# omerbt/Splice

Hardware: AMD Instinct MI355X
Metric: opt_steps_per_sec (higher is better)
Workload: dtype bf16

## Files before the change

### splice_amd/csrc/attn_bwd_x32.h

```cpp
#pragma once

constexpr int BX_SLOTS = 4;
constexpr int BX_Q_LDS = BX_SLOTS * 2 * 8192;
constexpr int BX_KV_LDS = BX_SLOTS * (2 * 8192 + 512);

__device__ __forceinline__ int bx_swz(int row) { return (((row >> 1) & 1) << 2) | (((row >> 3) & 1) << 1) | ((row >> 2) & 1); }

struct BxFrag {
    int rowa[4];
    int tra[2][2];
    __device__ __forceinline__ BxFrag(int lane) {
        const int q32 = lane & 31, hi = lane >> 5;
#pragma unroll
        for (int ks = 0; ks < 4; ++ks) rowa[ks] = q32 * 64 + (((2 * ks + hi) ^ bx_swz(q32)) << 3);
        const int m = lane & 15, dg = (lane >> 4) & 1;
#pragma unroll
        for (int db = 0; db < 2; ++db)
#pragma unroll
            for (int sec = 0; sec < 2; ++sec) {
                const int row = 8 * sec + 4 * hi + (m >> 2);
                tra[db][sec] = row * 64 + (((4 * db + 2 * dg + ((m >> 1) & 1)) ^ bx_swz(row)) << 3) + (m & 1) * 4;
            }
    }
};
__device__ __forceinline__ u32x4 bx_tr(const bf16_t* tile, const BxFrag& f, int db, int off) {
    typedef __attribute__((address_space(3))) tr_v4s lds_v4s;
    const tr_v4s lo = __builtin_amdgcn_ds_read_tr16_b64_v4i16((lds_v4s*)(tile + f.tra[db][0] + off));
    const tr_v4s hh = __builtin_amdgcn_ds_read_tr16_b64_v4i16((lds_v4s*)(tile + f.tra[db][1] + off));
    const uint2 x = __builtin_bit_cast(uint2, lo), y = __builtin_bit_cast(uint2, hh);
    return u32x4{x.x, x.y, y.x, y.y};
}
__device__ __forceinline__ void bx_mfma_seed(f32x16_t& d, const u32x4& a, const u32x4& b, const f32x16_t& c) {
    asm volatile("v_mfma_f32_32x32x16_bf16 %0, %1, %2, %3" : "=&v"(d) : "v"(a), "v"(b), "v"(c));
}
#define BX_SB __builtin_amdgcn_sched_barrier(0)

template <int NW>
struct BxDma {
    static constexpr int PIECES = 8 / NW;
    int wave, lr, chunk;
    uint32_t off[PIECES];
    __device__ __forceinline__ BxDma(int lane, int wave_, int ld, int coldelta) : wave(wave_) {
        lr = lane >> 3;
        const int pos = lane & 7;
        chunk = pos ^ ((((lr >> 1) & 1) << 2) | ((wave & 1) << 1) | ((lr >> 2) & 1));
#pragma unroll
        for (int i = 0; i < PIECES; ++i) off[i] = (uint32_t)((((wave + NW * i) * 8 + lr) * ld + chunk * 8 + coldelta) * 2);
    }
    __device__ __forceinline__ void tile(const bf16_t* base, int ld, int coldelta, int row0, int rows_total, uint32_t dst) const {
        if (row0 + 64 <= rows_total) {
            const bf16_t* tb = base + (size_t)row0 * ld;
#pragma unroll
            for (int i = 0; i < PIECES; ++i) pp_dma16(dst + i * (NW * 1024), off[i], tb);
        } else {
#pragma unroll
            for (int i = 0; i < PIECES; ++i) {
                int t = row0 + (wave + NW * i) * 8 + lr;
                t = t < rows_total ? t : rows_total - 1;
                pp_dma16(dst + i * (NW * 1024), (uint32_t)((t * ld + chunk * 8 + coldelta) * 2), base);
            }
        }
    }
};

template <int NW, bool FOLD>
__device__ __forceinline__ void attn_bwd_q_x32_body(const AttnArgs& a, int xb, int h, int b, bf16_t* bx_smem ) {
    constexpr int NL = 2 * (8 / NW);
    const int lane = threadIdx.x & 63, q32 = lane & 31, hi = lane >> 5;
    const int wave = __builtin_amdgcn_readfirstlane(threadIdx.x >> 6);
    const int ld = 3 * a.D;
    const int qbase = xb * (32 * NW) + wave * 32;
    const bool active = qbase < a.Tld;
    const bf16_t* pbase = a.qkv + (size_t)b * a.Tld * ld + h * 64;
    const int nt = (a.T + 63) / 64;
    const BxDma<NW> dk_(lane, wave, ld, a.D), dv_(lane, wave, ld, 2 * a.D);
    const BxFrag fr(lane);
    const uint32_t lds0 = (uint32_t)(size_t)(__attribute__((address_space(3))) bf16_t*)bx_smem + (uint32_t)wave * 1024u;
    auto issue = [&](int tile, int slot) __attribute__((always_inline)) {
        const uint32_t dst = __builtin_amdgcn_readfirstlane(lds0 + (uint32_t)slot * 16384u);
        dk_.tile(pbase, ld, a.D, tile * 64, a.Tld, dst);
        dv_.tile(pbase, ld, 2 * a.D, tile * 64, a.Tld, dst + 8192u);
    };
    issue(0, 0);
    if (nt > 1) issue(1, 1);
    if (nt > 2) issue(2, 2);

    const int qidx = qbase + q32;
    const int qc = qidx < a.Tld ? qidx : a.Tld - 1;
    u32x4 qf[4], dof[4];
    {
        const bf16_t* pq = pbase + (size_t)qc * ld + hi * 8;
        const bf16_t* pd = a.dout + ((size_t)b * a.Tld + qc) * a.D + h * 64 + hi * 8;
#pragma unroll
        for (int ks = 0; ks < 4; ++ks) { qf[ks] = ld16v(pq + ks * 16); dof[ks] = ld16v(pd + ks * 16); }
    }
    const float lse_q = a.lse[((size_t)b * a.H + h) * a.Tld + qc];
    const float del_q = a.delta[((size_t)b * a.H + h) * a.Tld + qc];
    const float c2 = a.scale * LOG2E;
    f32x16_t negl, negd, dq[2], s[2], dp[2];
    const f32x16_t zero16 = {0.f, 0.f, 0.f, 0.f, 0.f, 0.f, 0.f, 0.f, 0.f, 0.f, 0.f, 0.f, 0.f, 0.f, 0.f, 0.f};
#pragma unroll
    for (int r = 0; r < 16; ++r) { negl[r] = -lse_q; negd[r] = -del_q; dq[0][r] = dq[1][r] = 0.f; s[0][r] = s[1][r] = dp[0][r] = dp[1][r] = 0.f; }
    u32x4 kf[4], vf[4];
    auto read_rows = [&](const bf16_t* K, int blk) __attribute__((always_inline)) {
#pragma unroll
        for (int ks = 0; ks < 4; ++ks) { kf[ks] = lds16(K + fr.rowa[ks] + blk * 2048); vf[ks] = lds16(K + 4096 + fr.rowa[ks] + blk * 2048); }
    };
    auto sdp = [&](f32x16_t& sx, f32x16_t& dx, int ks) __attribute__((always_inline)) {
        if (ks == 0) {
            if (FOLD) bx_mfma_seed(sx, kf[0], qf[0], negl); else sx = mfma32(kf[0], qf[0], zero16);
            bx_mfma_seed(dx, vf[0], dof[0], negd);
        } else { sx = mfma32(kf[ks], qf[ks], sx); dx = mfma32(vf[ks], dof[ks], dx); }
    };
    pp_wait_dma<0>();
    asm volatile("" : "+v"(qf[0]), "+v"(qf[1]), "+v"(qf[2]), "+v"(qf[3]), "+v"(dof[0]), "+v"(dof[1]), "+v"(dof[2]), "+v"(dof[3]));
    pp_barrier();
    if (active) {
        read_rows(bx_smem, 0);
#pragma unroll
        for (int ks = 0; ks < 4; ++ks) sdp(s[0], dp[0], ks);
        read_rows(bx_smem, 1);
    }
    int slot = 0;
    auto body = [&](auto TAILC, int t) __attribute__((always_inline)) {
        constexpr bool TAIL = decltype(TAILC)::value;
        const int s1 = (slot + 1) & 3, s3 = (slot + 3) & 3;
        if (!TAIL || t + 2 < nt) pp_wait_dma<NL>(); else pp_wait_dma<0>();
        asm volatile("s_waitcnt lgkmcnt(0)" ::: "memory");
        pp_barrier();
        if (!TAIL || t + 3 < nt) issue(t + 3, s3);
        if (active) {
            const bf16_t* Kt = bx_smem + slot * 8192;
            const bf16_t* Kn = bx_smem + s1 * 8192;
#pragma unroll
            for (int blk = 0; blk < 2; ++blk) {
                f32x16_t& sc = s[blk];
                f32x16_t& dc = dp[blk];
                f32x16_t& sn = s[blk ^ 1];
                f32x16_t& dn = dp[blk ^ 1];
                if (TAIL && t * 64 + 64 > a.T) {
#pragma unroll
                    for (int r = 0; r < 16; ++r) sc[r] = t * 64 + 32 * blk + 8 * (r >> 2) + 4 * hi + (r & 3) < a.T ? sc[r] : NEG_BIG;
                }
                float g[16];
                u32x4 dsb[2], ktf[2][2];
                auto va = [&](int r0, int n) __attribute__((always_inline)) {
#pragma unroll
                    for (int r = r0; r < r0 + n; ++r) {
                        const float p = FOLD ? __builtin_amdgcn_exp2f(sc[r]) : __builtin_amdgcn_exp2f(__builtin_fmaf(sc[r], c2, -lse_q));
                        g[r] = p * dc[r];
                    }
                    asm volatile("" : "+v"(g[r0]), "+v"(g[r0 + n - 1]));
                };
                auto cv = [&](int kk) __attribute__((always_inline)) {
                    const float* pp = &g[kk * 8];
                    dsb[kk] = u32x4{pack2bf(pp[0], pp[1]), pack2bf(pp[2], pp[3]), pack2bf(pp[4], pp[5]), pack2bf(pp[6], pp[7])};
                    pp_opaque(dsb[kk]);
                };
                auto rt = [&](int kk, int db) __attribute__((always_inline)) {
                    ktf[kk][db] = bx_tr(Kt, fr, db, blk * 2048 + kk * 1024);
                };
                BX_SB;
                sdp(sn, dn, 0); BX_SB; va(0, 4); rt(0, 0); BX_SB;
                sdp(sn, dn, 1); BX_SB; va(4, 4); cv(0); rt(0, 1); BX_SB;
                sdp(sn, dn, 2); BX_SB; va(8, 4); rt(1, 0); BX_SB;
                sdp(sn, dn, 3); BX_SB; va(12, 4); cv(1); rt(1, 1); BX_SB;
                const bf16_t* Kr = blk == 0 ? Kn : Kn;
#pragma unroll
                for (int kk = 0; kk < 2; ++kk)
#pragma unroll
                    for (int db = 0; db < 2; ++db) {
                        dq[db] = mfma32(ktf[kk][db], dsb[kk], dq[db]);
                        BX_SB;
                        const int ks = kk * 2 + db;
                        kf[ks] = lds16(Kr + fr.rowa[ks] + blk * 2048); vf[ks] = lds16(Kr + 4096 + fr.rowa[ks] + blk * 2048);
                        BX_SB;
                    }
            }
        }
        slot = s1;
    };
    {
        std::false_type MAIN; std::true_type TAILT;
        int t = 0;
        for (; t + 4 < nt; ++t) body(MAIN, t);
        for (; t < nt; ++t) body(TAILT, t);
    }
    if (!active || qidx >= a.Tld) return;
    bf16_t* op = a.dqkv + ((size_t)b * a.Tld + qidx) * ld + h * 64 + hi * 4;
#pragma unroll
    for (int db = 0; db < 2; ++db)
#pragma unroll
        for (int j = 0; j < 4; ++j)
            *reinterpret_cast<uint2*>(op + db * 32 + j * 8) = uint2{pack2bf(dq[db][4 * j] * a.scale, dq[db][4 * j + 1] * a.scale),
                                                                    pack2bf(dq[db][4 * j + 2] * a.scale, dq[db][4 * j + 3] * a.scale)};
}

template <int NW>
__device__ __forceinline__ void attn_bwd_kv_x32_body(const AttnArgs& a, int xb, int h, int b, bf16_t* bx_smem ) {
    constexpr int SLOT = 2 * 4096 + 256;
    static_assert(NW >= 2, "waves 0 and 1 move the lse / delta rows");
    const int lane = threadIdx.x & 63, k32 = lane & 31, hi = lane >> 5;
    const int wave = __builtin_amdgcn_readfirstlane(threadIdx.x >> 6);
    const int ld = 3 * a.D;
    const int kbase = xb * (32 * NW) + wave * 32;
    const bool active = kbase < a.Tld;
    const bf16_t* pbase = a.qkv + (size_t)b * a.Tld * ld + h * 64;
    const bf16_t* dobase = a.dout + (size_t)b * a.Tld * a.D + h * 64;
    const float* lse = a.lse + ((size_t)b * a.H + h) * a.Tld;
    const float* dl = a.delta + ((size_t)b * a.H + h) * a.Tld;
    const int nblk = a.Tld / 32, nt = (nblk + 1) / 2;
    const BxDma<NW> dq_(lane, wave, ld, 0), dd_(lane, wave, a.D, 0);
    const BxFrag fr(lane);
    const uint32_t ldsb = (uint32_t)(size_t)(__attribute__((address_space(3))) bf16_t*)bx_smem;
    const uint32_t lds0 = ldsb + (uint32_t)wave * 1024u;
    auto issue = [&](int tile, int slot) __attribute__((always_inline)) {
        const uint32_t dst = __builtin_amdgcn_readfirstlane(lds0 + (uint32_t)slot * (SLOT * 2));
        dq_.tile(pbase, ld, 0, tile * 64, a.Tld, dst);
        dd_.tile(dobase, a.D, 0, tile * 64, a.Tld, dst + 8192u);
        if (wave < 2) {
            const int r = tile * 64 + lane;
            const uint32_t voff = (uint32_t)((r < a.Tld ? r : a.Tld - 1) * 4);
            const uint32_t d2 = __builtin_amdgcn_readfirstlane(ldsb + (uint32_t)slot * (SLOT * 2) + 16384u + (uint32_t)wave * 256u);
            const float* src = wave == 0 ? lse : dl;
            asm volatile("s_mov_b32 m0, %0\n\ts_nop 0\n\tglobal_load_lds_dword %1, %2" ::"s"(d2), "v"(voff), "s"(src) : "memory");
        }
    };
    issue(0, 0);
    if (nt > 1) issue(1, 1);
    if (nt > 2) issue(2, 2);

    const int kidx = kbase + k32;
    const int kc = kidx < a.Tld ? kidx : a.Tld - 1;
    u32x4 kn[4], vn[4];
    {
        const bf16_t* pk = pbase + (size_t)kc * ld + a.D + hi * 8;
        const bf16_t* pv = pbase + (size_t)kc * ld + 2 * a.D + hi * 8;
#pragma unroll
        for (int ks = 0; ks < 4; ++ks) {
            kn[ks] = ld16v(pk + ks * 16); vn[ks] = ld16v(pv + ks * 16);
#pragma unroll
            for (int j = 0; j < 4; ++j) { kn[ks][j] ^= 0x80008000u; vn[ks][j] ^= 0x80008000u; }
        }
    }
    f32x16_t dkn[2], dv[2];
#pragma unroll
    for (int r = 0; r < 16; ++r) { dkn[0][r] = dkn[1][r] = dv[0][r] = dv[1][r] = 0.f; }
    u32x4 qr[4], dr[4];
    f32x16_t sx, dx;
    auto seeds = [&](const bf16_t* st, int blk) __attribute__((always_inline)) {
        const float* Ls = reinterpret_cast<const float*>(st + 8192);
#pragma unroll
        for (int j = 0; j < 4; ++j) {
            const f32x4 lv = *reinterpret_cast<const f32x4*>(Ls + 32 * blk + 8 * j + 4 * hi);
            const f32x4 ev = *reinterpret_cast<const f32x4*>(Ls + 64 + 32 * blk + 8 * j + 4 * hi);
#pragma unroll
            for (int i = 0; i < 4; ++i) { sx[4 * j + i] = lv[i]; dx[4 * j + i] = ev[i]; }
        }
    };
    auto rows = [&](const bf16_t* st, int blk) __attribute__((always_inline)) {
#pragma unroll
        for (int ks = 0; ks < 4; ++ks) { qr[ks] = lds16(st + fr.rowa[ks] + blk * 2048); dr[ks] = lds16(st + 4096 + fr.rowa[ks] + blk * 2048); }
    };
    pp_wait_dma<0>();
    asm volatile("" : "+v"(kn[0]), "+v"(kn[1]), "+v"(kn[2]), "+v"(kn[3]), "+v"(vn[0]), "+v"(vn[1]), "+v"(vn[2]), "+v"(vn[3]));
    pp_barrier();
    if (active) { rows(bx_smem, 0); seeds(bx_smem, 0); }
    int slot = 0;
    auto body = [&](auto TAILC, int t) __attribute__((always_inline)) {
        constexpr bool TAIL = decltype(TAILC)::value;
        const int s1 = (slot + 1) & 3, s3 = (slot + 3) & 3;
        if (!TAIL || t + 2 < nt) { if (wave < 2) pp_wait_dma<2 * (8 / NW) + 1>(); else pp_wait_dma<2 * (8 / NW)>(); } else pp_wait_dma<0>();
        asm volatile("s_waitcnt lgkmcnt(0)" ::: "memory");
        pp_barrier();
        if (!TAIL || t + 3 < nt) issue(t + 3, s3);
        if (active) {
            const bf16_t* st = bx_smem + slot * SLOT;
            const bf16_t* sn = bx_smem + s1 * SLOT;
#pragma unroll
            for (int blk = 0; blk < 2; ++blk) {
                if (TAIL && 2 * t + blk >= nblk) break;
                u32x4 dot[2][2], qt[2][2], pb[2], gb[2];
                float p[16], g[16];
#pragma unroll
                for (int ks = 0; ks < 4; ++ks) {
                    sx = mfma32(qr[ks], kn[ks], sx);
                    BX_SB;
                    {
                        if (ks < 2) { dot[ks][0] = bx_tr(st + 4096, fr, 0, blk * 2048 + ks * 1024); dot[ks][1] = bx_tr(st + 4096, fr, 1, blk * 2048 + ks * 1024); }
                        else { qt[ks - 2][0] = bx_tr(st, fr, 0, blk * 2048 + (ks - 2) * 1024); qt[ks - 2][1] = bx_tr(st, fr, 1, blk * 2048 + (ks - 2) * 1024); }
                    }
                    BX_SB;
                }
#pragma unroll
                for (int ks = 0; ks < 4; ++ks) {
                    dx = mfma32(dr[ks], vn[ks], dx);
                    BX_SB;
                    {
#pragma unroll
                        for (int r = 4 * ks; r < 4 * ks + 4; ++r) p[r] = __builtin_amdgcn_exp2f(-sx[r]);
                        if (ks & 1) {
                            const float* pp = &p[(ks >> 1) * 8];
                            pb[ks >> 1] = u32x4{pack2bf(pp[0], pp[1]), pack2bf(pp[2], pp[3]), pack2bf(pp[4], pp[5]), pack2bf(pp[6], pp[7])};
                            pp_opaque(pb[ks >> 1]);
                        } else asm volatile("" : "+v"(p[4 * ks]), "+v"(p[4 * ks + 3]));
                    }
                    BX_SB;
                }
#pragma unroll
                for (int i4 = 0; i4 < 4; ++i4) {
                    const int kk = i4 >> 1, db = i4 & 1;
                    dv[db] = mfma32(dot[kk][db], pb[kk], dv[db]);
                    BX_SB;
                    {
#pragma unroll
                        for (int r = 4 * i4; r < 4 * i4 + 4; ++r) g[r] = p[r] * dx[r];
                        if (i4 & 1) {
                            const float* pp = &g[(i4 >> 1) * 8];
                            gb[i4 >> 1] = u32x4{pack2bf(pp[0], pp[1]), pack2bf(pp[2], pp[3]), pack2bf(pp[4], pp[5]), pack2bf(pp[6], pp[7])};
                            pp_opaque(gb[i4 >> 1]);
                        } else asm volatile("" : "+v"(g[4 * i4]), "+v"(g[4 * i4 + 3]));
                    }
                    BX_SB;
                }
                const bf16_t* nx_st = blk == 0 ? st : sn;
                const int nx_blk = blk ^ 1;
#pragma unroll
                for (int i4 = 0; i4 < 4; ++i4) {
                    const int kk = i4 >> 1, db = i4 & 1;
                    dkn[db] = mfma32(qt[kk][db], gb[kk], dkn[db]);
                    BX_SB;
                    {
                        const float* Ls = reinterpret_cast<const float*>(nx_st + 8192);
                        qr[i4] = lds16(nx_st + fr.rowa[i4] + nx_blk * 2048);
                        dr[i4] = lds16(nx_st + 4096 + fr.rowa[i4] + nx_blk * 2048);
                        const f32x4 lv = *reinterpret_cast<const f32x4*>(Ls + 32 * nx_blk + 8 * i4 + 4 * hi);
                        const f32x4 ev = *reinterpret_cast<const f32x4*>(Ls + 64 + 32 * nx_blk + 8 * i4 + 4 * hi);
#pragma unroll
                        for (int i = 0; i < 4; ++i) { sx[4 * i4 + i] = lv[i]; dx[4 * i4 + i] = ev[i]; }
                    }
                    BX_SB;
                }
            }
        }
        slot = s1;
    };
    {
        std::false_type MAIN; std::true_type TAILT;
        int t = 0;
        for (; t + 4 < nt; ++t) body(MAIN, t);
        for (; t < nt; ++t) body(TAILT, t);
    }
    if (!active || kidx >= a.Tld) return;
    const float sk = kidx < a.T ? -a.scale : 0.f, sv = kidx < a.T ? 1.0f : 0.f;
    bf16_t* pk = a.dqkv + ((size_t)b * a.Tld + kidx) * ld + a.D + h * 64 + hi * 4;
    bf16_t* pv = a.dqkv + ((size_t)b * a.Tld + kidx) * ld + 2 * a.D + h * 64 + hi * 4;
#pragma unroll
    for (int db = 0; db < 2; ++db)
#pragma unroll
        for (int j = 0; j < 4; ++j) {
            *reinterpret_cast<uint2*>(pk + db * 32 + j * 8) = uint2{pack2bf(dkn[db][4 * j] * sk, dkn[db][4 * j + 1] * sk), pack2bf(dkn[db][4 * j + 2] * sk, dkn[db][4 * j + 3] * sk)};
            *reinterpret_cast<uint2*>(pv + db * 32 + j * 8) = uint2{pack2bf(dv[db][4 * j] * sv, dv[db][4 * j + 1] * sv), pack2bf(dv[db][4 * j + 2] * sv, dv[db][4 * j + 3] * sv)};
        }
}
#undef BX_SB

template <int NW>
__global__ __launch_bounds__(64 * NW) void attn_bwd_x32_kernel(AttnArgs a, int nx) {
    extern __shared__ __attribute__((aligned(16))) bf16_t bx_smem[];
    const int n = nx * a.H * a.B;
    const int lid = xcd_remap(blockIdx.x, 2 * n);
    const int pair = lid >> 1;
    const int xb = pair % nx, bh = pair / nx;
    const int h = bh % a.H, b = bh / a.H;
    if (lid & 1) attn_bwd_kv_x32_body<NW>(a, xb, h, b, bx_smem);
    else attn_bwd_q_x32_body<NW, true>(a, xb, h, b, bx_smem);
}
template <int NW>
__global__ __launch_bounds__(64 * NW) void attn_bwd_q_x32_kernel(AttnArgs a, int nx) {
    extern __shared__ __attribute__((aligned(16))) bf16_t bx_smem[];
    int xb, h, b;
    attn_block_coords(nx, a.H, a.B, xb, h, b);
    attn_bwd_q_x32_body<NW, true>(a, xb, h, b, bx_smem);
}
template <int NW>
__global__ __launch_bounds__(64 * NW) void attn_bwd_kv_x32_kernel(AttnArgs a, int nx) {
    extern __shared__ __attribute__((aligned(16))) bf16_t bx_smem[];
    int xb, h, b;
    attn_block_coords(nx, a.H, a.B, xb, h, b);
    attn_bwd_kv_x32_body<NW>(a, xb, h, b, bx_smem);
}
```

### splice_amd/csrc/attn_x32.h

```cpp
#pragma once
#include <type_traits>

template <int NW>
struct X32 {
    static constexpr int PIECES = 8 / NW;
    static constexpr int NL = 2 * PIECES;
    static constexpr int LDS_BYTES = 6 * 8192;
};

__device__ __forceinline__ void pp_dma16(uint32_t lds_byte, uint32_t voff, const void* sbase) {
    asm volatile("s_mov_b32 m0, %0\n\ts_nop 0\n\tglobal_load_lds_dwordx4 %1, %2" ::"s"(lds_byte), "v"(voff), "s"(sbase) : "memory");
}
template <int N>
__device__ __forceinline__ void pp_wait_dma() { asm volatile("s_waitcnt vmcnt(%0)" ::"n"(N) : "memory"); }
__device__ __forceinline__ void pp_barrier() {
    __builtin_amdgcn_sched_barrier(0);
    __builtin_amdgcn_s_barrier();
    __builtin_amdgcn_sched_barrier(0);
}
template <class V> __device__ __forceinline__ void pp_opaque(V& v) { asm volatile("" : "+v"(v)); }

typedef __attribute__((ext_vector_type(16))) float f32x16_t;
__device__ __forceinline__ f32x16_t mfma32(const u32x4& a, const u32x4& b, const f32x16_t& c) {
    return __builtin_amdgcn_mfma_f32_32x32x16_bf16(__builtin_bit_cast(bf16x8, a), __builtin_bit_cast(bf16x8, b), c, 0, 0, 0);
}
__device__ __forceinline__ float half2_max(float v) { return fmaxf(v, __shfl_xor(v, 32, 64)); }

__device__ __forceinline__ void x32_exact_rows(const AttnArgs& a, const bf16_t* pbase, int b, int h, int qidx, int hi, float c2) {
    const int ld = 3 * a.D;
    const int qc = qidx < a.Tld ? qidx : a.Tld - 1;
    float q[64], o[64];
    {
        const bf16_t* p = pbase + (size_t)qc * ld;
#pragma unroll
        for (int i = 0; i < 8; ++i) {
            const u32x4 v = ld16v(p + i * 8);
#pragma unroll
            for (int j = 0; j < 4; ++j) { q[i * 8 + 2 * j] = __uint_as_float(v[j] << 16) * c2; q[i * 8 + 2 * j + 1] = __uint_as_float(v[j] & 0xFFFF0000u) * c2; }
        }
    }
#pragma unroll
    for (int d = 0; d < 64; ++d) o[d] = 0.f;
    float m = NEG_BIG, l = 0.f;
    for (int key = hi; key < a.T; key += 2) {
        const bf16_t* kp = pbase + (size_t)key * ld + a.D;
        float sc = 0.f;
#pragma unroll
        for (int i = 0; i < 8; ++i) {
            const u32x4 v = ld16v(kp + i * 8);
#pragma unroll
            for (int j = 0; j < 4; ++j) {
                sc = __builtin_fmaf(q[i * 8 + 2 * j], __uint_as_float(v[j] << 16), sc);
                sc = __builtin_fmaf(q[i * 8 + 2 * j + 1], __uint_as_float(v[j] & 0xFFFF0000u), sc);
            }
        }
        const float mn = fmaxf(m, sc);
        const float alpha = __builtin_amdgcn_exp2f(m - mn), pk = __builtin_amdgcn_exp2f(sc - mn);
        m = mn;
        l = l * alpha + pk;
        const bf16_t* vp = pbase + (size_t)key * ld + 2 * a.D;
#pragma unroll
        for (int i = 0; i < 8; ++i) {
            const u32x4 v = ld16v(vp + i * 8);
#pragma unroll
            for (int j = 0; j < 4; ++j) {
                o[i * 8 + 2 * j] = __builtin_fmaf(pk, __uint_as_float(v[j] << 16), o[i * 8 + 2 * j] * alpha);
                o[i * 8 + 2 * j + 1] = __builtin_fmaf(pk, __uint_as_float(v[j] & 0xFFFF0000u), o[i * 8 + 2 * j + 1] * alpha);
            }
        }
    }
    const float m1 = __shfl_xor(m, 32, 64), l1 = __shfl_xor(l, 32, 64);
    const float mn = fmaxf(m, m1);
    const float a0 = __builtin_amdgcn_exp2f(m - mn), a1 = __builtin_amdgcn_exp2f(m1 - mn);
    const float lt = l * a0 + l1 * a1, inv = 1.0f / lt;
    bf16_t* op = a.out + ((size_t)b * a.Tld + qc) * a.D + h * 64;
#pragma unroll
    for (int d = 0; d < 64; ++d) {
        const float od = (o[d] * a0 + __shfl_xor(o[d], 32, 64) * a1) * inv;
        if (hi == (d >> 5) && qidx < a.Tld) op[d] = f2bf(od);
    }
    if (hi == 0 && qidx < a.Tld) a.lse[((size_t)b * a.H + h) * a.Tld + qidx] = mn + __builtin_amdgcn_logf(lt);
}

template <int NW, bool FOLD>
__global__ __launch_bounds__(64 * NW) void attn_fwd_x32_kernel(AttnArgs a, int nx) {
    extern __shared__ __attribute__((aligned(16))) bf16_t x32_smem[];
    constexpr int PIECES = X32<NW>::PIECES, NL = X32<NW>::NL;
    const int lane = threadIdx.x & 63;
    const int q32 = lane & 31, hi = lane >> 5;
    const int wave = __builtin_amdgcn_readfirstlane(threadIdx.x >> 6);
    int xb, h, b;
    attn_block_coords(nx, a.H, a.B, xb, h, b);
    const int ld = 3 * a.D;
    const int qbase = xb * (32 * NW) + wave * 32;
    const bool active = qbase < a.Tld;
    const bf16_t* pbase = a.qkv + (size_t)b * a.Tld * ld + h * 64;
    const int nt = (a.T + 63) / 64;

    const int lr = lane >> 3, pos = lane & 7;
    const int kchunk = pos ^ (((wave & 1) << 2) | (lr >> 1));
    const int vchunk = pos ^ (((lr >> 1) & 1) << 2);
    uint32_t koffs[PIECES], voffs[PIECES];
#pragma unroll
    for (int i = 0; i < PIECES; ++i) {
        const int row = (wave + NW * i) * 8 + lr;
        koffs[i] = (uint32_t)((row * ld + kchunk * 8 + a.D) * 2);
        voffs[i] = (uint32_t)((row * ld + vchunk * 8 + 2 * a.D) * 2);
    }
    const uint32_t lds0 = (uint32_t)(size_t)(__attribute__((address_space(3))) bf16_t*)x32_smem + (uint32_t)wave * 1024u;
    auto issue_tile = [&](const uint32_t (&offs)[PIECES], int chunk, int coldelta, int tile, uint32_t dst) __attribute__((always_inline)) {
        const int kt = tile * 64;
        if (kt + 64 <= a.Tld) {
            const bf16_t* tb = pbase + (size_t)kt * ld;
#pragma unroll
            for (int i = 0; i < PIECES; ++i) pp_dma16(dst + i * (NW * 1024), offs[i], tb);
        } else {
#pragma unroll
            for (int i = 0; i < PIECES; ++i) {
                int t = kt + (wave + NW * i) * 8 + lr;
                t = t < a.Tld ? t : a.Tld - 1;
                pp_dma16(dst + i * (NW * 1024), (uint32_t)((t * ld + chunk * 8 + coldelta) * 2), pbase);
            }
        }
    };
    auto issue_k = [&](int tile, int slot) __attribute__((always_inline)) { issue_tile(koffs, kchunk, a.D, tile, __builtin_amdgcn_readfirstlane(lds0 + (uint32_t)slot * 8192u)); };
    auto issue_v = [&](int tile, int slot) __attribute__((always_inline)) { issue_tile(voffs, vchunk, 2 * a.D, tile, __builtin_amdgcn_readfirstlane(lds0 + 3 * 8192u + (uint32_t)slot * 8192u)); };
    const char* kptr = reinterpret_cast<const char*>(pbase) + (size_t)4 * 64 * ld * 2;
    const char* vptr = reinterpret_cast<const char*>(pbase) + (size_t)2 * 64 * ld * 2;
    const size_t tile_bytes = (size_t)64 * ld * 2;
    auto issue_fast = [&](int s1, int s2) __attribute__((always_inline)) {
        const uint32_t kd = __builtin_amdgcn_readfirstlane(lds0 + (uint32_t)s1 * 8192u), vd = __builtin_amdgcn_readfirstlane(lds0 + 3 * 8192u + (uint32_t)s2 * 8192u);
#pragma unroll
        for (int i = 0; i < PIECES; ++i) pp_dma16(kd + i * (NW * 1024), koffs[i], kptr);
#pragma unroll
        for (int i = 0; i < PIECES; ++i) pp_dma16(vd + i * (NW * 1024), voffs[i], vptr);
    };
    issue_k(0, 0);
    issue_v(0, 0);
    if (nt > 1) { issue_k(1, 1); issue_v(1, 1); }
    if (nt > 2) issue_k(2, 2);

    u32x4 qf[4];
    const int qidx = qbase + q32;
    {
        const int qc = qidx < a.Tld ? qidx : a.Tld - 1;
        const bf16_t* p = pbase + (size_t)qc * ld + hi * 8;
#pragma unroll
        for (int ks = 0; ks < 4; ++ks) qf[ks] = ld16v(p + ks * 16);
    }
    int ka[4];
#pragma unroll
    for (int ks = 0; ks < 4; ++ks) ka[ks] = q32 * 64 + (((2 * ks + hi) ^ ((q32 >> 1) & 7)) << 3);
    int va[2];
    {
        const int m = lane & 15, dg = (lane >> 4) & 1;
#pragma unroll
        for (int db = 0; db < 2; ++db)
            va[db] = (4 * hi + (m >> 2)) * 64 + (((4 * db + 2 * dg + ((m >> 1) & 1)) ^ (((m >> 3) & 1) << 2)) << 3) + (m & 1) * 4;
    }
    float m_ref = 0.f, l = 0.f;
    f32x16_t o[2], sb[2][2], negm;
#pragma unroll
    for (int r = 0; r < 16; ++r) { o[0][r] = 0.f; o[1][r] = 0.f; sb[0][0][r] = sb[0][1][r] = sb[1][0][r] = sb[1][1][r] = 0.f; negm[r] = 0.f; }
    const float c2 = a.scale * LOG2E;
    const f32x16_t zero16 = {0.f, 0.f, 0.f, 0.f, 0.f, 0.f, 0.f, 0.f, 0.f, 0.f, 0.f, 0.f, 0.f, 0.f, 0.f, 0.f};
    u32x4 kf[2][4];
    auto read_k = [&](const bf16_t* Ks) __attribute__((always_inline)) {
#pragma unroll
        for (int kb = 0; kb < 2; ++kb)
#pragma unroll
            for (int ks = 0; ks < 4; ++ks) kf[kb][ks] = lds16(Ks + ka[ks] + kb * 2048);
    };
    auto scores = [&](f32x16_t (&s)[2], const f32x16_t& seed) __attribute__((always_inline)) {
#pragma unroll
        for (int kb = 0; kb < 2; ++kb) s[kb] = mfma32(kf[kb][0], qf[0], seed);
#pragma unroll
        for (int ks = 1; ks < 4; ++ks)
#pragma unroll
            for (int kb = 0; kb < 2; ++kb) s[kb] = mfma32(kf[kb][ks], qf[ks], s[kb]);
    };
    const bf16_t* Kring = x32_smem;
    const bf16_t* Vring = x32_smem + 3 * 4096;

    pp_wait_dma<0>();
    asm volatile("" : "+v"(qf[0]), "+v"(qf[1]), "+v"(qf[2]), "+v"(qf[3]));
    pp_barrier();
    if (active) {
        read_k(Kring);
        scores(sb[0], zero16);
        float mx = NEG_BIG;
#pragma unroll
        for (int kb = 0; kb < 2; ++kb)
#pragma unroll
            for (int r = 0; r < 16; ++r) {
                const bool valid = 32 * kb + 8 * (r >> 2) + 4 * hi + (r & 3) < a.T;
                mx = fmaxf(mx, valid ? sb[0][kb][r] : NEG_BIG);
            }
        m_ref = half2_max(mx) * (FOLD ? 1.0f : c2);
#pragma unroll
        for (int r = 0; r < 16; ++r) negm[r] = -m_ref;
        if (FOLD) scores(sb[0], negm);
        if (nt > 1) read_k(Kring + 4096);
    }
    asm volatile("s_waitcnt lgkmcnt(0)" ::: "memory");
    pp_barrier();
    if (nt > 3) issue_k(3, 0);

    int slot = 0;
#define X32_SB __builtin_amdgcn_sched_barrier(0)
    auto body = [&](auto PARC, auto TAILC, int t) __attribute__((always_inline)) {
        constexpr int PAR = decltype(PARC)::value;
        constexpr bool TAIL = decltype(TAILC)::value;
        f32x16_t (&s)[2] = sb[PAR];
        f32x16_t (&sn)[2] = sb[PAR ^ 1];
        const int s1 = slot == 2 ? 0 : slot + 1, s2 = slot == 0 ? 2 : slot - 1;
        if (!TAIL || t + 3 < nt) pp_wait_dma<NL>(); else pp_wait_dma<0>();
        asm volatile("s_waitcnt lgkmcnt(0)" ::: "memory");
        pp_barrier();
        if (!TAIL) issue_fast(s1, s2);
        else {
            if (t + 4 < nt) issue_k(t + 4, s1);
            if (t + 2 < nt) issue_v(t + 2, s2);
        }
        kptr += tile_bytes;
        vptr += tile_bytes;
        if (active) {
            const bf16_t* Vs = Vring + slot * 4096;
            const bf16_t* Kn = Kring + s2 * 4096;
            u32x4 vf[4][2], pb[4];
            float p[2][16];
            float pa[4] = {0.f, 0.f, 0.f, 0.f};
            const int kt = t * 64;
            if (TAIL && kt + 64 > a.T) {
#pragma unroll
                for (int kb = 0; kb < 2; ++kb)
#pragma unroll
                    for (int r = 0; r < 16; ++r) s[kb][r] = kt + 32 * kb + 8 * (r >> 2) + 4 * hi + (r & 3) < a.T ? s[kb][r] : NEG_BIG;
            }
            auto ex = [&](int kb, int r0, int n) __attribute__((always_inline)) {
#pragma unroll
                for (int r = r0; r < r0 + n; ++r) {
                    p[kb][r] = FOLD ? __builtin_amdgcn_exp2f(s[kb][r]) : __builtin_amdgcn_exp2f(__builtin_fmaf(s[kb][r], c2, -m_ref));
                    pa[r & 3] += p[kb][r];
                }
                asm volatile("" : "+v"(pa[0]), "+v"(pa[1]), "+v"(pa[2]), "+v"(pa[3]));
            };
            auto cv = [&](int kk) __attribute__((always_inline)) {
                const float* pp = &p[kk >> 1][(kk & 1) * 8];
                pb[kk] = u32x4{pack2bf(pp[0], pp[1]), pack2bf(pp[2], pp[3]), pack2bf(pp[4], pp[5]), pack2bf(pp[6], pp[7])};
                pp_opaque(pb[kk]);
            };
            auto rv = [&](int kk, int db) __attribute__((always_inline)) {
                typedef __attribute__((address_space(3))) tr_v4s lds_v4s;
                const tr_v4s lo = __builtin_amdgcn_ds_read_tr16_b64_v4i16((lds_v4s*)(Vs + va[db] + kk * 1024));
                const tr_v4s hh = __builtin_amdgcn_ds_read_tr16_b64_v4i16((lds_v4s*)(Vs + va[db] + kk * 1024 + 512));
                const uint2 x = __builtin_bit_cast(uint2, lo), y = __builtin_bit_cast(uint2, hh);
                vf[kk][db] = u32x4{x.x, x.y, y.x, y.y};
            };
            auto rk = [&](int kb, int ks) __attribute__((always_inline)) {
                kf[kb][ks] = lds16(Kn + ka[ks] + kb * 2048);
            };
            auto qk = [&](int kb, int ks) __attribute__((always_inline)) {
                if (ks == 0 && FOLD) asm volatile("v_mfma_f32_32x32x16_bf16 %0, %1, %2, %3" : "=&v"(sn[kb]) : "v"(kf[kb][0]), "v"(qf[0]), "v"(negm));
                else sn[kb] = mfma32(kf[kb][ks], qf[ks], ks == 0 ? zero16 : sn[kb]);
            };
            auto pv = [&](int kk, int db) __attribute__((always_inline)) {
                o[db] = mfma32(vf[kk][db], pb[kk], o[db]);
            };
            X32_SB;
            qk(0, 0); X32_SB; ex(0, 0, 3); rv(0, 0); X32_SB;
            qk(1, 0); X32_SB; ex(0, 3, 3); rv(0, 1); X32_SB;
            qk(0, 1); X32_SB; ex(0, 6, 2); cv(0); rv(1, 0); X32_SB;
            qk(1, 1); X32_SB; ex(0, 8, 3); rv(1, 1); X32_SB;
            qk(0, 2); X32_SB; ex(0, 11, 3); rv(2, 0); X32_SB;
            qk(1, 2); X32_SB; ex(0, 14, 2); cv(1); rv(2, 1); X32_SB;
            qk(0, 3); X32_SB; ex(1, 0, 3); rv(3, 0); X32_SB;
            qk(1, 3); X32_SB; ex(1, 3, 3); rv(3, 1); X32_SB;
            pv(0, 0); X32_SB; ex(1, 6, 2); cv(2); rk(0, 0); X32_SB;
            pv(0, 1); X32_SB; ex(1, 8, 3); rk(1, 0); X32_SB;
            pv(1, 0); X32_SB; ex(1, 11, 3); rk(0, 1); X32_SB;
            pv(1, 1); X32_SB; ex(1, 14, 2); cv(3); rk(1, 1); X32_SB;
            pv(2, 0); X32_SB; rk(0, 2); X32_SB;
            pv(2, 1); X32_SB; rk(1, 2); X32_SB;
            pv(3, 0); X32_SB; rk(0, 3); X32_SB;
            pv(3, 1); X32_SB; rk(1, 3); X32_SB;
            const float ps = (pa[0] + pa[1]) + (pa[2] + pa[3]);
            l += ps;
            if (__builtin_expect(__any(!(ps < ATTN_RESCALE_LIMIT)), 0)) {
                const bool mine = half2_max(!(ps < ATTN_RESCALE_LIMIT) ? 1.0f : 0.0f) > 0.f;
                const float lq = l + __shfl_xor(l, 32, 64);
                const float shift = mine ? __builtin_amdgcn_logf(lq) : 0.f;
                const float alpha = __builtin_amdgcn_exp2f(-shift);
                m_ref += shift;
                l *= alpha;
#pragma unroll
                for (int r = 0; r < 16; ++r) {
                    negm[r] = -m_ref; o[0][r] *= alpha; o[1][r] *= alpha;
                    if (FOLD) { sn[0][r] -= shift; sn[1][r] -= shift; }
                }
            }
        }
        slot = s1;
    };
    {
        std::integral_constant<int, 0> P0; std::integral_constant<int, 1> P1;
        std::false_type MAIN; std::true_type TAILT;
        int t = 0;
        for (; t + 6 < nt; t += 2) {
            body(P0, MAIN, t);
            body(P1, MAIN, t + 1);
        }
        for (; t < nt; t += 2) {
            body(P0, TAILT, t);
            if (t + 1 < nt) body(P1, TAILT, t + 1);
        }
    }
#undef X32_SB
    if (!active) return;
    const float lt = l + __shfl_xor(l, 32, 64);
    if (__builtin_expect(__any(!(lt > 0.25f && lt < 1.0e37f)), 0)) {
        x32_exact_rows(a, pbase, b, h, qidx, hi, FOLD ? 1.0f : c2);
        return;
    }
    if (qidx < a.Tld) {
        const float inv = 1.0f / lt;
        bf16_t* op = a.out + ((size_t)b * a.Tld + qidx) * a.D + h * 64 + hi * 4;
#pragma unroll
        for (int db = 0; db < 2; ++db)
#pragma unroll
            for (int j = 0; j < 4; ++j)
                *reinterpret_cast<uint2*>(op + db * 32 + j * 8) =
                    uint2{pack2bf(o[db][4 * j] * inv, o[db][4 * j + 1] * inv), pack2bf(o[db][4 * j + 2] * inv, o[db][4 * j + 3] * inv)};
        if (hi == 0) a.lse[((size_t)b * a.H + h) * a.Tld + qidx] = m_ref + __builtin_amdgcn_logf(lt);
    }
}
```

Measured before the change: 263.5.

## Widen attention output stores via permlane swap and overlap Q load with K/V DMA

```diff
diff --git a/splice_amd/csrc/attn_bwd_x32.h b/splice_amd/csrc/attn_bwd_x32.h
--- a/splice_amd/csrc/attn_bwd_x32.h
+++ b/splice_amd/csrc/attn_bwd_x32.h
@@ -186,14 +186,8 @@
         for (; t + 4 < nt; ++t) body(MAIN, t);
         for (; t < nt; ++t) body(TAILT, t);
     }
-    if (!active || qidx >= a.Tld) return;
-    bf16_t* op = a.dqkv + ((size_t)b * a.Tld + qidx) * ld + h * 64 + hi * 4;
-#pragma unroll
-    for (int db = 0; db < 2; ++db)
-#pragma unroll
-        for (int j = 0; j < 4; ++j)
-            *reinterpret_cast<uint2*>(op + db * 32 + j * 8) = uint2{pack2bf(dq[db][4 * j] * a.scale, dq[db][4 * j + 1] * a.scale),
-                                                                    pack2bf(dq[db][4 * j + 2] * a.scale, dq[db][4 * j + 3] * a.scale)};
+    if (!active) return;
+    pp_store_row(a.dqkv + ((size_t)b * a.Tld + qidx) * ld + h * 64 + hi * 8, dq, a.scale, qidx < a.Tld);
 }
 
 template <int NW>
@@ -351,17 +345,11 @@
         for (; t + 4 < nt; ++t) body(MAIN, t);
         for (; t < nt; ++t) body(TAILT, t);
     }
-    if (!active || kidx >= a.Tld) return;
+    if (!active) return;
     const float sk = kidx < a.T ? -a.scale : 0.f, sv = kidx < a.T ? 1.0f : 0.f;
-    bf16_t* pk = a.dqkv + ((size_t)b * a.Tld + kidx) * ld + a.D + h * 64 + hi * 4;
-    bf16_t* pv = a.dqkv + ((size_t)b * a.Tld + kidx) * ld + 2 * a.D + h * 64 + hi * 4;
-#pragma unroll
-    for (int db = 0; db < 2; ++db)
-#pragma unroll
-        for (int j = 0; j < 4; ++j) {
-            *reinterpret_cast<uint2*>(pk + db * 32 + j * 8) = uint2{pack2bf(dkn[db][4 * j] * sk, dkn[db][4 * j + 1] * sk), pack2bf(dkn[db][4 * j + 2] * sk, dkn[db][4 * j + 3] * sk)};
-            *reinterpret_cast<uint2*>(pv + db * 32 + j * 8) = uint2{pack2bf(dv[db][4 * j] * sv, dv[db][4 * j + 1] * sv), pack2bf(dv[db][4 * j + 2] * sv, dv[db][4 * j + 3] * sv)};
-        }
+    bf16_t* pk = a.dqkv + ((size_t)b * a.Tld + kidx) * ld + a.D + h * 64 + hi * 8;
+    pp_store_row(pk, dkn, sk, kidx < a.Tld);
+    pp_store_row(pk + a.D, dv, sv, kidx < a.Tld);
 }
 #undef BX_SB
 
diff --git a/splice_amd/csrc/attn_x32.h b/splice_amd/csrc/attn_x32.h
--- a/splice_amd/csrc/attn_x32.h
+++ b/splice_amd/csrc/attn_x32.h
@@ -25,6 +25,32 @@
     return __builtin_amdgcn_mfma_f32_32x32x16_bf16(__builtin_bit_cast(bf16x8, a), __builtin_bit_cast(bf16x8, b), c, 0, 0, 0);
 }
 __device__ __forceinline__ float half2_max(float v) { return fmaxf(v, __shfl_xor(v, 32, 64)); }
+
+template <int OFF>
+__device__ __forceinline__ void pp_gload16(u32x4& d, const void* p) { asm volatile("global_load_dwordx4 %0, %1, off offset:%2" : "=v"(d) : "v"(p), "n"(OFF) : "memory"); }
+__device__ __forceinline__ void pp_gload16x4(u32x4 (&d)[4], const void* p) {
+    pp_gload16<0>(d[0], p); pp_gload16<32>(d[1], p); pp_gload16<64>(d[2], p); pp_gload16<96>(d[3], p);
+}
+template <int N>
+__device__ __forceinline__ void pp_wait_regs(u32x4 (&r)[4]) {
+    asm volatile("s_waitcnt vmcnt(%4)" : "+v"(r[0]), "+v"(r[1]), "+v"(r[2]), "+v"(r[3]) : "n"(N) : "memory");
+}
+__device__ __forceinline__ u32x4 pp_row16(uint2 lo, uint2 hh) {
+    const auto x = __builtin_amdgcn_permlane32_swap(lo.x, hh.x, false, false);
+    const auto y = __builtin_amdgcn_permlane32_swap(lo.y, hh.y, false, false);
+    return u32x4{x[0], y[0], x[1], y[1]};
+}
+__device__ __forceinline__ void pp_store_row(bf16_t* p, const f32x16_t (&o)[2], float s, bool live) {
+#pragma unroll
+    for (int db = 0; db < 2; ++db)
+#pragma unroll
+        for (int jp = 0; jp < 2; ++jp) {
+            const int r = 8 * jp;
+            const u32x4 w = pp_row16(uint2{pack2bf(o[db][r] * s, o[db][r + 1] * s), pack2bf(o[db][r + 2] * s, o[db][r + 3] * s)},
+                                     uint2{pack2bf(o[db][r + 4] * s, o[db][r + 5] * s), pack2bf(o[db][r + 6] * s, o[db][r + 7] * s)});
+            if (live) *reinterpret_cast<u32x4*>(p + db * 32 + jp * 16) = w;
+        }
+}
 
 __device__ __forceinline__ void x32_exact_rows(const AttnArgs& a, const bf16_t* pbase, int b, int h, int qidx, int hi, float c2) {
     const int ld = 3 * a.D;
@@ -135,19 +161,16 @@
 #pragma unroll
         for (int i = 0; i < PIECES; ++i) pp_dma16(vd + i * (NW * 1024), voffs[i], vptr);
     };
+    u32x4 qf[4];
+    const int qidx = qbase + q32;
+    {
+        const int qc = qidx < a.Tld ? qidx : a.Tld - 1;
+        pp_gload16x4(qf, pbase + (size_t)qc * ld + hi * 8);
+    }
     issue_k(0, 0);
     issue_v(0, 0);
     if (nt > 1) { issue_k(1, 1); issue_v(1, 1); }
     if (nt > 2) issue_k(2, 2);
-
-    u32x4 qf[4];
-    const int qidx = qbase + q32;
-    {
-        const int qc = qidx < a.Tld ? qidx : a.Tld - 1;
-        const bf16_t* p = pbase + (size_t)qc * ld + hi * 8;
-#pragma unroll
-        for (int ks = 0; ks < 4; ++ks) qf[ks] = ld16v(p + ks * 16);
-    }
     int ka[4];
 #pragma unroll
     for (int ks = 0; ks < 4; ++ks) ka[ks] = q32 * 64 + (((2 * ks + hi) ^ ((q32 >> 1) & 7)) << 3);
@@ -182,8 +205,8 @@
     const bf16_t* Kring = x32_smem;
     const bf16_t* Vring = x32_smem + 3 * 4096;
 
-    pp_wait_dma<0>();
-    asm volatile("" : "+v"(qf[0]), "+v"(qf[1]), "+v"(qf[2]), "+v"(qf[3]));
+    if (nt > 2) pp_wait_dma<4 * PIECES>(); else if (nt > 1) pp_wait_dma<3 * PIECES>(); else pp_wait_dma<PIECES>();
+    pp_wait_regs<4 * PIECES>(qf);
     pp_barrier();
     if (active) {
         read_k(Kring);
@@ -200,11 +223,13 @@
 #pragma unroll
         for (int r = 0; r < 16; ++r) negm[r] = -m_ref;
         if (FOLD) scores(sb[0], negm);
-        if (nt > 1) read_k(Kring + 4096);
-    }
+    }
+    if (nt > 2) pp_wait_dma<2 * PIECES>(); else pp_wait_dma<PIECES>();
     asm volatile("s_waitcnt lgkmcnt(0)" ::: "memory");
     pp_barrier();
     if (nt > 3) issue_k(3, 0);
+    if (active && nt > 1) read_k(Kring + 4096);
+    if (nt > 3) pp_wait_dma<PIECES>(); else pp_wait_dma<0>();
 
     int slot = 0;
 #define X32_SB __builtin_amdgcn_sched_barrier(0)
@@ -322,15 +347,7 @@
         x32_exact_rows(a, pbase, b, h, qidx, hi, FOLD ? 1.0f : c2);
         return;
     }
-    if (qidx < a.Tld) {
-        const float inv = 1.0f / lt;
-        bf16_t* op = a.out + ((size_t)b * a.Tld + qidx) * a.D + h * 64 + hi * 4;
-#pragma unroll
-        for (int db = 0; db < 2; ++db)
-#pragma unroll
-            for (int j = 0; j < 4; ++j)
-                *reinterpret_cast<uint2*>(op + db * 32 + j * 8) =
-                    uint2{pack2bf(o[db][4 * j] * inv, o[db][4 * j + 1] * inv), pack2bf(o[db][4 * j + 2] * inv, o[db][4 * j + 3] * inv)};
-        if (hi == 0) a.lse[((size_t)b * a.H + h) * a.Tld + qidx] = m_ref + __builtin_amdgcn_logf(lt);
-    }
-}
+    const float inv = 1.0f / lt;
+    pp_store_row(a.out + ((size_t)b * a.Tld + qidx) * a.D + h * 64 + hi * 8, o, inv, qidx < a.Tld);
+    if (qidx < a.Tld && hi == 0) a.lse[((size_t)b * a.H + h) * a.Tld + qidx] = m_ref + __builtin_amdgcn_logf(lt);
+}
```

Result: no change. 265.6, median of 6 (+0.8%).
